# sean-lo/OptimalMatrixCompletion.jl

Measured on AMD Instinct MI355X. Metric: B&B node-relaxations/sec, 100x100 k=1, higher is better.
Workload: dtype f64

## Files before the change

optimalmatrixcompletion.jl_amd/csrc/omc_api.cpp:

```cpp
#include <hip/hip_runtime.h>
#include <stdint.h>
#include <limits.h>
#include <stdio.h>
#include <stdlib.h>
#include <string.h>
#include <math.h>
#include <chrono>
#include <string>
#include <vector>
#include <algorithm>
#include <atomic>
#include <thread>
#include <mutex>

#include "omc.h"
#include "omc_device.h"
#include "omc_altmin.h"
#include "omc_shor.h"
#include "omc_shor_relax.h"
#include <unordered_map>
#include <dlfcn.h>
#include <execinfo.h>
#include <signal.h>
#include <unistd.h>
// ... 35 lines not shown
  p->eps_gap = 1e-6; p->eps_feas = 1e-7; p->max_iters = 3000; p->check_every = 25;
  p->rho_scale = 1.0; p->rho_f_ratio = 0.1; p->relax = 1.6; p->time_limit = 3600.0;
  p->reference_quirk_q1 = 1; p->breakpoints = OMC_SMALLEST_1_EIGVEC; p->stall_checks = 8;
  p->bump_max = 2; p->bump_ratio = 4.0; p->bump_factor = 4.0; p->bump_after = 100; p->bump_window = 4; p->slots = 0;
  p->accel = 0; p->aa_mem = 10; p->aa_every = 10; p->aa_start = 50; p->aa_reg = 1e-10; p->aa_safeguard = 1.0; p->first_wins = 0;
  p->early_stop_after = 400; p->early_stop_factor = 1.5;
}

static int upload(DevBuf& b, const void* src, size_t bytes, hipStream_t s) {
  int rc = b.ensure(bytes ? bytes : 8);
  if (rc) return rc;
  if (bytes) HIPCHK(hipMemcpyAsync(b.p, src, bytes, hipMemcpyHostToDevice, s));
  return 0;
}

static int build_colprox_lists(omc_instance* h, int block_min, bool pair_on) {
  if (h->lists_valid && h->lists_block_min == block_min && h->lists_pair == pair_on) return 0;
  const int m = h->m, lds_c = cp_block_lds_cmax(), max_c = cp_block_cmax();
  std::vector<int> solo, wide, blk, slab;
  std::vector<uint8_t> isb(m, 0);
  h->cpb_cl = h->cpb_cs = h->crest_max = h->nrest = 0;
  for (int j0 = 0; j0 < m; j0 += 2) {
    const int j1 = j0 + 1;
    const int c0 = h->col_ptr[j0 + 1] - h->col_ptr[j0], c1 = (j1 < m) ? h->col_ptr[j1 + 1] - h->col_ptr[j1] : 0;
    const bool paired = j1 < m && c0 <= 32 && c1 <= 32;
    for (int j = j0; j <= j1 && j < m; ++j) {
      const int c = (j == j0) ? c0 : c1;
      if (c == 0) continue;
      if (!(paired && pair_on) && c >= block_min && c <= max_c) {
        isb[j] = 1;
        if (c <= lds_c) { blk.push_back(j); h->cpb_cl = std::max(h->cpb_cl, c); } else { slab.push_back(j); h->cpb_cs = std::max(h->cpb_cs, c); }
        continue;
      }
      ++h->nrest; h->crest_max = std::max(h->crest_max, c);
      if (paired) continue;
      if (c <= 64) wide.push_back(j); else solo.push_back(j);
    }
  }
  h->nsolo = (int)solo.size(); h->nwide = (int)wide.size(); h->nblock = (int)blk.size(); h->nslab = (int)slab.size();
  int rc = 0;
  if (h->nsolo && (rc = upload(h->dsolo, solo.data(), sizeof(int) * solo.size(), h->stream))) return rc;
  if (h->nwide && (rc = upload(h->dwide, wide.data(), sizeof(int) * wide.size(), h->stream))) return rc;
  if (h->nblock && (rc = upload(h->dblock, blk.data(), sizeof(int) * blk.size(), h->stream))) return rc;
  if (h->nslab && (rc = upload(h->dslab, slab.data(), sizeof(int) * slab.size(), h->stream))) return rc;
  if ((rc = upload(h->disblock, isb.data(), (size_t)m, h->stream))) return rc;
  HIPCHK(hipStreamSynchronize(h->stream));
  h->lists_valid = true; h->lists_block_min = block_min; h->lists_pair = pair_on;
  return 0;
}

int omc_instance_create(int n, int m, int k, const double* A, const uint8_t* mask, double gamma, int device,
                        omc_instance** out) {
  if (!out) return fail(OMC_ERR_ARGUMENT, "out is NULL");
  *out = nullptr;
  if (!A || !mask) return fail(OMC_ERR_ARGUMENT, "A / mask is NULL");
  if (n <= 0 || m <= 0) return fail(OMC_ERR_DIMENSION, "Dimension mismatch: A must have size (n, m) (OMC.jl:240-246)");
  if (!(n <= m)) return fail(OMC_ERR_DIMENSION, "Input matrix A must have size (n, m) with n <= m (OMC.jl:249-254)");
  if (k < 1 || k > n) return fail(OMC_ERR_ARGUMENT, "rank k must satisfy 1 <= k <= n");
  if (k > 8) return fail(OMC_ERR_UNSUPPORTED, "k > 8 is not supported by this build");
  if (!(gamma > 0.0)) return fail(OMC_ERR_ARGUMENT, "gamma must be positive");
  int ndev = 0;
  if (hipGetDeviceCount(&ndev) != hipSuccess || ndev <= 0)
// ... 28 lines not shown
  h->row_ptr.assign(n + 1, 0);
  for (int i = 0; i < n; ++i) {
    int c = 0;
    for (int j = 0; j < m; ++j)
      if (h->mask[(size_t)j * n + i]) { h->row_idx.push_back(j); h->row_val.push_back(A[(size_t)j * n + i]); ++c; }
    h->row_ptr[i + 1] = h->row_ptr[i] + c;
  }
  HIPCHK(hipStreamCreate(&h->stream));
  int rc = 0;
  if ((rc = upload(h->drow_ptr, h->row_ptr.data(), sizeof(int) * (n + 1), h->stream))) return rc;
  if ((rc = upload(h->drow_idx, h->row_idx.data(), sizeof(int) * h->nnz_rows(), h->stream))) return rc;
  if ((rc = upload(h->drow_val, h->row_val.data(), sizeof(double) * h->nnz_rows(), h->stream))) return rc;
  if ((rc = upload(h->dA, h->A.data(), sizeof(double) * n * m, h->stream))) return rc;
  if ((rc = upload(h->dmask, h->mask.data(), (size_t)n * m, h->stream))) return rc;
  if ((rc = upload(h->dcol_ptr, h->col_ptr.data(), sizeof(int) * (m + 1), h->stream))) return rc;
  if ((rc = build_colprox_lists(h, h->tun.colprox_block_min, !h->tun.no_colprox_pair))) return rc;
  if ((rc = upload(h->dcol_idx, h->col_idx.data(), sizeof(int) * h->nnz, h->stream))) return rc;
  if ((rc = upload(h->dcol_val, h->col_val.data(), sizeof(double) * h->nnz, h->stream))) return rc;
  if ((rc = upload(h->dNcnt, h->Ncnt.data(), sizeof(double) * n * n, h->stream))) return rc;
  HIPCHK(hipStreamSynchronize(h->stream));
  int lrc = omc_set_max_lds();
  if (lrc) return fail(lrc, "hipFuncSetAttribute(MaxDynamicSharedMemorySize) failed");
  { int arc = omc_altmin_set_lds(); if (arc) return fail(5000 + arc, "hipFuncSetAttribute(MaxDynamicSharedMemorySize) failed for the altmin kernel"); }
  omc_relax_params_default(&h->params);
  *out = h;
  h = nullptr;
  return 0;
}

int omc_instance_create_bits(int n, int m, int k, const double* A, const uint64_t* chunks, double gamma, int device,
                             omc_instance** out) {
// ... 261 lines not shown
    int r0 = h->bgap.ensure(sizeof(double) * 2 * (size_t)S); if (r0) return r0;
    r0 = h->bvotes.ensure(sizeof(int) * (size_t)S); if (r0) return r0;
    r0 = h->bslotlist.ensure(sizeof(int) * (size_t)S); if (r0) return r0;
    w.gap_prev = h->bgap.as<double>(); w.gap_rate = h->bgap.as<double>() + S; w.slow_votes = h->bvotes.as<int>();
    w.slot_list = nullptr;
  }
  std::vector<double> wY((size_t)n * n);
  for (size_t e = 0; e < (size_t)n * n; ++e) wY[e] = shor ? 3.0 : P.rho_f_ratio * h->Ncnt[e] + 2.0;
  int rc_ = 0;
  if ((rc_ = upload(h->dwY, wY.data(), sizeof(double) * n * n, h->stream))) return rc_;
  w.col_ptr = h->dcol_ptr.as<int>(); w.col_idx = h->dcol_idx.as<int>(); w.col_val = h->dcol_val.as<double>();
  const int cp_force = h->cp_force;
  h->cp_force = 0;
  {
    const bool pair_on = !h->tun.no_colprox_pair && cp_force != 2;
    if ((rc_ = build_colprox_lists(h, cp_force == 1 ? INT_MAX : cp_force == 2 ? 1 : h->tun.colprox_block_min, pair_on))) return rc_;
    w.cp_pair = pair_on ? 1 : 0;
  }
  w.cp_nblock = h->nblock; w.cp_block = h->nblock ? h->dblock.as<int>() : nullptr;
  w.cp_nslab = h->nslab; w.cp_slab = h->nslab ? h->dslab.as<int>() : nullptr;
  w.cp_isblock = (h->nblock + h->nslab) ? h->disblock.as<unsigned char>() : nullptr; w.cp_nrest = h->nrest; w.cp_nfact = nullptr;
  w.cone_512 = h->tun.cone_512 ? 1 : 0; w.cp_series = CP_SERIES; w.cp_maxpass = CP_MAXPASS; w.cp_xcd = h->tun.colprox_no_xcd ? 0 : 1;
  w.cp_nsolo = h->nsolo; w.cp_solo = h->nsolo ? h->dsolo.as<int>() : nullptr;
  w.cp_nwide = h->nwide; w.cp_wide = h->nwide ? h->dwide.as<int>() : nullptr;
  w.Ncnt = h->dNcnt.as<double>(); w.wY1 = h->dwY.as<double>();
  w.row_ptr = h->drow_ptr.as<int>(); w.row_idx = h->drow_idx.as<int>();
#define ENS(buf, bytes) do { int r_ = (buf).ensure(bytes); if (r_) return r_; } while (0)
  const size_t sB = (size_t)S;
  const size_t sN = (size_t)B + (size_t)extra_nodes;
  ENS(h->bY, sB * n * n * 8); ENS(h->bYp, sB * n * n * 8); ENS(h->bU, sB * n * k * 8);
  ENS(h->bD1, sB * n * n * 8); ENS(h->bD3, sB * n * n * 8); ENS(h->bW1, sB * n * n * 8); ENS(h->bE3, sB * n * n * 8);
  ENS(h->bdS, sB * rmax * rmax * 8);
// ... 1864 lines not shown
```

optimalmatrixcompletion.jl_amd/csrc/omc_colprox.hip:

```cpp
#include <hip/hip_runtime.h>
#include <type_traits>
#include <stdint.h>
#include "omc_device.h"
#include "omc_wave.h"

template <int Q>
__device__ __forceinline__ double half_bcast(double v) {
  int lo = __double2loint(v), hi = __double2hiint(v);
  lo = __builtin_amdgcn_update_dpp(0, lo, 0x150 + (Q & 15), 0xF, 0xF, false);
  hi = __builtin_amdgcn_update_dpp(0, hi, 0x150 + (Q & 15), 0xF, 0xF, false);
  auto a = __builtin_amdgcn_permlane16_swap(lo, lo, false, false);
  auto c = __builtin_amdgcn_permlane16_swap(hi, hi, false, false);
  return (Q < 16) ? __hiloint2double(c[0], a[0]) : __hiloint2double(c[1], a[1]);
}
__device__ __forceinline__ double half_sum(double v) {
  v = group_sum_dpp<16>(v);
  const int lo = __double2loint(v), hi = __double2hiint(v);
  auto a = __builtin_amdgcn_permlane16_swap(lo, lo, false, false);
  auto c = __builtin_amdgcn_permlane16_swap(hi, hi, false, false);
  return __hiloint2double(c[0], a[0]) + __hiloint2double(c[1], a[1]);
}
#define CPP_LDS_DOUBLES (64 + 64 + 32)

template <int LPC>
__device__ __forceinline__ double lanes_sum(double v) { if constexpr (LPC == 32) return half_sum(v); else return wave_sum(v); }
#define RQ(q) (((q) < 32) ? R0[(q) & 31] : R1[((NC > 32) ? (q) : 0) & 31])
typedef double dbl2_lds __attribute__((ext_vector_type(2), may_alias));
template <int LPC>
__device__ __forceinline__ void colprox_sweep(const OmcWS& w, const int b, const int lane, const int j, const int off, const int c, const int cmax,
                                              double* st, double* vo_s, int* sidx) {
  constexpr int NC = LPC;
  const int h = (LPC == 32) ? (lane >> 5) : 0, l = lane & (LPC - 1), hb = h * LPC;
  const bool act = l < c;
  const int n = w.n;
  const double gm = w.gamma;
  const double* Y = w.Y + (size_t)b * n * n;
  const double* Yp = w.Yp + (size_t)b * n * n;
  const double* Yx = w.Yx ? w.Yx + (size_t)b * n * n : nullptr;
  double* alpha = w.alpha + (size_t)b * w.nnz + off;
  const double a_reg = act ? w.col_val[off + l] : 0.0;
  const int my = act ? w.col_idx[off + l] : 0;
  const double vo_r = act ? alpha[l] : 0.0;
  sidx[lane] = my; vo_s[lane] = vo_r;
  const double rho_f = w.rho_b[b] * w.rho_f_ratio;
  const double coef = gm / (2.0 * rho_f), cp = gm * gm / (2.0 * rho_f);
  double R0[32], R1[(NC > 32) ? 32 : 1], sc;
  const dbl2_lds* st2 = (const dbl2_lds*)st;
  auto gather = [&](double shift) __attribute__((always_inline)) {
#pragma unroll
    for (int qb = 0; qb < NC; qb += 8) {
      if (qb < cmax) {
        double y1[8], y2[8], vq[8];
#pragma unroll
        for (int u = 0; u < 8; ++u) {
          const int iq = sidx[hb + qb + u];
          vq[u] = vo_s[hb + qb + u];
          const size_t a = (l > qb + u) ? (size_t)iq * n + my : (size_t)my * n + iq;
          y1[u] = Yx ? Yx[a] : Y[a]; y2[u] = Yx ? 0.0 : Yp[a];
        }
#pragma unroll
        for (int u = 0; u < 8; ++u) {
          const int q = qb + u;
          const double v = gm * ((Yx ? y1[u] : 2.0 * y1[u] - y2[u]) - coef * vo_r * vq[u]);
          RQ(q) = (l == q) ? (act ? v + 1.0 : 1.0) + shift : ((act && q < c) ? v : 0.0);
        }
      } else {
#pragma unroll
        for (int u = 0; u < 8; ++u) RQ(qb + u) = 0.0;
      }
    }
  };
  auto invert = [&]() __attribute__((always_inline)) -> bool {
    int cm = cmax;
    asm volatile("" : "+s"(cm));
    int lv = l;
    asm volatile("" : "+v"(lv));
    sc = 1.0;
    double isc = 1.0;
    bool good = true;
#pragma unroll
    for (int k = 0; k < NC; ++k) {
      if (k < cm) {
        const double ak = RQ(k) * sc;
        st[lane] = ak;
        const double d = st[hb + k];
        good = good && (d > 1e-290);
        const double pinv = fast_rcp(d);
        const bool piv = (lv == k);
        const double tt = piv ? 0.0 : ak * pinv * isc;
#pragma unroll
        for (int qb = 0; qb < NC; qb += 4) {
          if (qb < cm) {
            if constexpr (LPC == 32) {
              const dbl2_lds s01 = st2[(hb + qb) >> 1], s23 = st2[((hb + qb) >> 1) + 1];
              if (qb != k) RQ(qb) = fma(-tt, s01.x, RQ(qb));
              if (qb + 1 != k) RQ(qb + 1) = fma(-tt, s01.y, RQ(qb + 1));
              if (qb + 2 != k) RQ(qb + 2) = fma(-tt, s23.x, RQ(qb + 2));
              if (qb + 3 != k) RQ(qb + 3) = fma(-tt, s23.y, RQ(qb + 3));
            } else {
#pragma unroll
              for (int u = 0; u < 4; ++u) {
                const int q = qb + u;
                if (q != k) RQ(q) = fma(-tt, st[hb + q], RQ(q));
              }
            }
          }
        }
        RQ(k) = piv ? -1.0 : tt;
        sc = piv ? pinv : sc;
        isc = piv ? d : isc;
      }
    }
    return good;
  };
  auto apply = [&](double v) __attribute__((always_inline)) -> double {
    int cm = cmax;
    asm volatile("" : "+s"(cm));
    st[lane] = v;
    double a0 = 0.0, a1 = 0.0, a2 = 0.0, a3 = 0.0;
#pragma unroll
    for (int qb = 0; qb < NC; qb += 4) {
      if (qb < cm) {
        if constexpr (LPC == 32) {
          const dbl2_lds s01 = st2[(hb + qb) >> 1], s23 = st2[((hb + qb) >> 1) + 1];
          a0 = fma(RQ(qb), s01.x, a0); a1 = fma(RQ(qb + 1), s01.y, a1);
          a2 = fma(RQ(qb + 2), s23.x, a2); a3 = fma(RQ(qb + 3), s23.y, a3);
        } else {
          a0 = fma(RQ(qb), st[hb + qb], a0); a1 = fma(RQ(qb + 1), st[hb + qb + 1], a1);
          a2 = fma(RQ(qb + 2), st[hb + qb + 2], a2); a3 = fma(RQ(qb + 3), st[hb + qb + 3], a3);
        }
      }
    }
    return -sc * ((a0 + a1) + (a2 + a3));
  };
  const double sprev = (j < w.m) ? w.sval[(size_t)b * w.m + j] : 0.0;
  double s = (sprev > 0.0) ? sprev : 0.0;
  double lo = 0.0, hi = -1.0;
  bool lo_valid = false, fin = (c == 0);
  double yout = 0.0;
  const double ser_lim = (w.cp_series >= 6) ? 5e-3 : 1e-5;
  int npass = 0; double dr_first = -1.0; int why = 0;
  for (int it = 0; it <= 60; ++it) {
    if (!__any(!fin)) break;
    const bool last = (it >= w.cp_maxpass);
    gather(cp * s);
    const bool ok_ = invert();
    if (!fin) ++npass;
    double v[6] = {0.0, 0.0, 0.0, 0.0, 0.0, 0.0};
    double rhs = a_reg, yy = 0.0, yz = 0.0, zz = 0.0;
    bool want_ser = false; double dstep = 0.0;
    int K = 2;
    for (int sv = 0; sv < K; ++sv) {
      const double x = apply(rhs);
      rhs = x;
#pragma unroll
      for (int q = 0; q < 6; ++q) v[q] = (sv == q) ? x : v[q];
      if (sv == 0 && last) { if (!fin) { yout = x; fin = true; } break; }
      if (sv == 1) {
        yy = lanes_sum<LPC>(v[0] * v[0]); yz = lanes_sum<LPC>(v[0] * v[1]); zz = lanes_sum<LPC>(v[1] * v[1]);
        bool big = false;
        if (!fin) {
          if (!ok_) {
            lo = s; lo_valid = false;
            s = (hi > 0.0) ? 0.5 * (s + hi) : (2.0 * s + 1.0);
          } else {
            const double ph = yy - s, dph = -2.0 * cp * yz - 1.0, ddph = 6.0 * cp * cp * zz;
            if (ph >= 0.0) { lo = s; lo_valid = true; } else { hi = s; }
            const double den = 2.0 * dph * dph - ph * ddph;
            double sn = s + ((den > dph * dph) ? (-2.0 * ph * dph / den) : (-ph / dph));
            bool guarded = false;
            if (!(sn > lo) && !lo_valid) { sn = 0.5 * (lo + s); guarded = true; }
            if (sn < lo) { sn = lo; guarded = true; }
            if (hi > 0.0 && sn > hi) { sn = 0.5 * (lo + hi); guarded = true; }
            const double d = sn - s;
            const double dr = (yy > 0.0) ? cp * fabs(d) * sqrt(zz / yy) : 1.0;
            if (dr_first < 0.0) { dr_first = dr; why = guarded ? 1 : 0; }
            if (fabs(d) <= 1e-13 * fmax(1.0, fabs(s))) { fin = true; yout = v[0]; }
            else if (!guarded && dr < ser_lim) { want_ser = true; dstep = d; big = dr >= 1e-5; }
            else s = sn;
          }
        }
        if (__any(want_ser)) K = __any(want_ser && big) ? 6 : 3;
      }
    }
    if (K > 2) {
      double mo[13];
      mo[2] = yy; mo[3] = yz; mo[4] = zz;
#pragma unroll
      for (int i = 2; i < 6; ++i) {
        if (i < K) { mo[2 * i + 1] = lanes_sum<LPC>(v[i - 1] * v[i]); mo[2 * i + 2] = lanes_sum<LPC>(v[i] * v[i]); }
        else { mo[2 * i + 1] = 0.0; mo[2 * i + 2] = 0.0; }
      }
      if (want_ser) {
        double cf[11];
#pragma unroll
        for (int p = 2; p <= 12; ++p) {
          const int cnt = (p <= K + 1) ? p - 1 : ((p <= 2 * K) ? 2 * K - p + 1 : 0);
          cf[p - 2] = (double)cnt * mo[p];
        }
        double d = dstep;
        bool conv = false;
        for (int nt = 0; nt < 8; ++nt) {
          const double t = -cp * d;
          double G = 0.0, dG = 0.0;
#pragma unroll
          for (int q = 10; q >= 0; --q) { dG = fma(dG, t, G); G = fma(G, t, cf[q]); }
          const double F = G - s - d, dF = -cp * dG - 1.0;
          const double dn = d - F / dF;
          conv = fabs(dn - d) <= 1e-14 * fmax(fabs(s), fabs(dn));
          d = dn;
          if (conv) break;
        }
        const double t = cp * d;
        const double t2 = t * t;
        const double lastterm = ((K == 6) ? t2 * t2 * fabs(t) : t2) * sqrt(fmax((K == 6) ? mo[12] : mo[6], 0.0));
        const double growth = sqrt(fmax((K == 6) ? mo[12] : mo[6], 0.0) / fmax((K == 6) ? mo[10] : mo[4], 1e-300));
        if (conv && s + d > lo * (lo_valid ? 1.0 : 0.0) && lastterm * fabs(t) * growth <= 2e-15 * sqrt(yy) && fabs(t) * growth < 0.05) {
          double acc = 0.0;
#pragma unroll
          for (int q = 5; q >= 0; --q) acc = (q < K) ? fma(acc, -t, v[q]) : acc;
          yout = acc; s = s + d; fin = true;
        } else {
          s = s + dstep;
        }
      }
    }
  }
  if (w.sub_debug == 4 && l == 0 && c > 0) {
    atomicAdd(&w.stamps[(npass < 7) ? npass : 7], 1.0);
    if (dr_first >= 0.0) { const int bin = (dr_first > 0.0) ? (int)fmin(15.0, fmax(0.0, -log10(dr_first))) : 15; atomicAdd(&w.stamps[8 + bin], 1.0); if (why) atomicAdd(&w.stamps[24], 1.0); }
    else atomicAdd(&w.stamps[25], 1.0);
  }
  if (act) {
    alpha[l] = yout;
    w.lamD[((size_t)b * w.m + j) * n + my] = yout;
    if (l == 0) w.sval[(size_t)b * w.m + j] = s;
  }
}


#undef RQ
__global__ void __launch_bounds__(256) __attribute__((amdgpu_waves_per_eu(3))) k_colprox_pair(OmcWS w) {
  extern __shared__ double smem[];
  const int wave_in_blk = __builtin_amdgcn_readfirstlane(threadIdx.x >> 6), lane = threadIdx.x & 63, wpb = blockDim.x >> 6;
  const int gw = xcd_block(w.cp_xcd) * wpb + wave_in_blk;
  const int mp = (w.m + 1) >> 1;
  const int bl = gw / mp, pr = gw - bl * mp;
  if (bl >= w.nB) return;
  const int b = slot_of(w, bl);
  if (w.done[b]) return;
  const int j0 = 2 * pr, j1 = j0 + 1;
  const int off0 = w.col_ptr[j0], c0 = w.col_ptr[j0 + 1] - off0;
  const int off1 = (j1 < w.m) ? w.col_ptr[j1] : 0, c1 = (j1 < w.m) ? w.col_ptr[j1 + 1] - off1 : 0;
  if (c0 > 32 || c1 > 32 || j1 >= w.m) return;
  const int cmax = __builtin_amdgcn_readfirstlane((c0 > c1) ? c0 : c1);
  if (cmax == 0) return;
  double* st = smem + (size_t)wave_in_blk * CPP_LDS_DOUBLES;
  double* vo_s = st + 64;
  int* sidx = (int*)(vo_s + 64);
  const int h = lane >> 5;
  colprox_sweep<32>(w, b, lane, j0 + h, h ? off1 : off0, h ? c1 : c0, cmax, st, vo_s, sidx);
}

__global__ void __launch_bounds__(256) __attribute__((amdgpu_waves_per_eu(2))) k_colprox_wide(OmcWS w) {
  extern __shared__ double smem[];
  const int wave_in_blk = __builtin_amdgcn_readfirstlane(threadIdx.x >> 6), lane = threadIdx.x & 63, wpb = blockDim.x >> 6;
  const int gw = xcd_block(w.cp_xcd) * wpb + wave_in_blk;
  const int bl = gw / w.cp_nwide, jj = gw - bl * w.cp_nwide;
  if (bl >= w.nB) return;
  const int b = slot_of(w, bl);
  if (w.done[b]) return;
  const int j = w.cp_wide[jj];
  const int off = w.col_ptr[j], c = w.col_ptr[j + 1] - off;
  const int cmax = __builtin_amdgcn_readfirstlane(c);
  if (cmax == 0 || cmax > 64) return;
  double* st = smem + (size_t)wave_in_blk * CPP_LDS_DOUBLES;
  double* vo_s = st + 64;
  int* sidx = (int*)(vo_s + 64);
  colprox_sweep<64>(w, b, lane, j, off, c, cmax, st, vo_s, sidx);
}


extern "C" void omc_launch_colprox_sweep(const OmcWS* w, hipStream_t s) {
  const int wpb = 4;
  const int wp = w->nB * ((w->m + 1) / 2);
  hipLaunchKernelGGL(k_colprox_pair, dim3((wp + wpb - 1) / wpb), dim3(wpb * 64), (size_t)wpb * CPP_LDS_DOUBLES * sizeof(double), s, *w);
  if (w->cp_nwide > 0) {
    const int ww = w->nB * w->cp_nwide;
    hipLaunchKernelGGL(k_colprox_wide, dim3((ww + wpb - 1) / wpb), dim3(wpb * 64), (size_t)wpb * CPP_LDS_DOUBLES * sizeof(double), s, *w);
  }
}

extern "C" void omc_colprox_sweep_residency(int* pair, int* wide) {
  const int wpb = 4;
  const size_t lds = (size_t)wpb * CPP_LDS_DOUBLES * sizeof(double);
  if (hipOccupancyMaxActiveBlocksPerMultiprocessor(pair, (const void*)k_colprox_pair, wpb * 64, lds) != hipSuccess) *pair = -1;
  if (hipOccupancyMaxActiveBlocksPerMultiprocessor(wide, (const void*)k_colprox_wide, wpb * 64, lds) != hipSuccess) *wide = -1;
}
```

optimalmatrixcompletion.jl_amd/csrc/omc_device.h:

```cpp
#ifndef OMC_DEVICE_H
#define OMC_DEVICE_H
#include <hip/hip_runtime.h>
#include <stdint.h>

#define ROW_TRACE 0
#define ROW_BOX 1
#define ROW_BOUND 2
#define ROW_CUT 3

#define CONE_CLIP01 0
#define CONE_EVALS 2
#define CONE_SEP 3
#define CONE_TOPK 4
#define CONE_BIG 5
#define SMALL_PROJ 0
#define SMALL_RECOVER 1

#define OMC_ST_OPTIMAL 0
#define OMC_ST_SLOW 1
#define OMC_ST_TIME 2
#define OMC_ST_INFEASIBLE 3

#include "omc_layout.h"

// ... 66 lines not shown
  int *rkind, *rcut, *rbi, *rbj;
  double* rcoef;
  double* rrhs;
  double* cutx;
  double* G;
  int setup_gram_inline;
  double* lam;
  double *obj, *objout, *objprev, *lbprev, *lb, *c0, *evsum, *cpen, *cst, *rp, *rd, *lmin;
  double* bx;
  int *done, *status, *iters, *sweeps, *stall;
  int* rowov;
  OmcGeom geo;
  double* cp_scratch;
  int cp_pair; int cp_nsolo; const int* cp_solo;
  int cp_nwide; const int* cp_wide;
  int cp_nrest;
  int cp_nblock, cp_nslab; const int *cp_block, *cp_slab; const unsigned char* cp_isblock; double* cp_bslab; int* cp_nfact;
  double* Yx;
  int cone_512;
  int cp_series;
  int cp_maxpass;
  int cp_xcd;
  double *cone_scratch, *glob_scratch, *small_scratch;
  double* chk_scratch;
  double* stamps;
  int accel, aa_mem, aa_every, aa_start, aa_dim;
  double aa_reg, aa_safeguard;
  double *aa_F, *aa_G, *aa_zin;
  double* aa_fn;
  int *aa_hist, *aa_head, *aa_pending, *aa_valid, *aa_nacc, *aa_nrej;
// ... 40 lines not shown
```

optimalmatrixcompletion.jl_amd/csrc/omc_host.h:

```cpp
#pragma once
#include <hip/hip_runtime.h>
#include <stdint.h>
#include <atomic>
#include <mutex>
#include <string>
#include <thread>
#include <unordered_map>
#include <vector>

#include "omc.h"
#include "omc_device.h"
#include "omc_shor_relax.h"

extern thread_local std::string g_err;
static inline int fail(int code, const std::string& msg) { g_err = msg; return code; }
#define HIPCHK(x)                                                                                         \
  do {                                                                                                    \
    hipError_t e_ = (x);                                                                                  \
    if (e_ != hipSuccess) {                                                                               \
      g_err = std::string(#x) + ": " + hipGetErrorString(e_);                                             \
      return (int)e_ > 0 ? (int)e_ : 999;                                                                 \
    }                                                                                                     \
  } while (0)

// ... 40 lines not shown
  bool colprox_no_xcd = false;
  bool cone_512 = false;
  bool dense_proj = false;
  bool host_phases = false;
  bool global_nolds = false;
  bool no_colprox_pair = false;
  bool no_graph = false;
  bool no_subspace = false;
  bool no_ws_split = false;
  bool segv_trace = false;
  bool setup_gram_inline = false;
  bool shor_explicit = false;
  bool shor_no_subspace = false;
  int check_xs = 16;
  int colprox_block_min = 65;
  int cone_multi_min = 1025;
  int graph_max = 16;
  int harvest_async = 1;
  int harvest_async_min_live = 256;
  int shor_select_kb = 1048576;
  int streams = 4;
  int sub_debug = 0;
  int sub_qmax = 24;
  int timing_stride = 1;
  int ws_quiet = 1;
};
struct Knob { const char* name; bool Tuning::*flag; int Tuning::*num; };
inline const Knob OMC_KNOBS[] = {
  {"OMC_ALTMIN_NOLDS", &Tuning::altmin_nolds, nullptr},      {"OMC_COLPROX_NO_XCD", &Tuning::colprox_no_xcd, nullptr},
  {"OMC_CONE_512", &Tuning::cone_512, nullptr},              {"OMC_DENSE_PROJ", &Tuning::dense_proj, nullptr},
  {"OMC_GLOBAL_NOLDS", &Tuning::global_nolds, nullptr},      {"OMC_HOST_PHASES", &Tuning::host_phases, nullptr},
  {"OMC_NO_COLPROX_PAIR", &Tuning::no_colprox_pair, nullptr},
  {"OMC_NO_GRAPH", &Tuning::no_graph, nullptr},              {"OMC_NO_SUBSPACE", &Tuning::no_subspace, nullptr},
  {"OMC_NO_WS_SPLIT", &Tuning::no_ws_split, nullptr},        {"OMC_SEGV_TRACE", &Tuning::segv_trace, nullptr},
  {"OMC_SETUP_GRAM_INLINE", &Tuning::setup_gram_inline, nullptr},
  {"OMC_SHOR_EXPLICIT", &Tuning::shor_explicit, nullptr},    {"OMC_SHOR_NO_SUBSPACE", &Tuning::shor_no_subspace, nullptr},
  {"OMC_COLPROX_BLOCK_MIN", nullptr, &Tuning::colprox_block_min},
  {"OMC_CHECK_XS", nullptr, &Tuning::check_xs},              {"OMC_CONE_MULTI_MIN", nullptr, &Tuning::cone_multi_min},
  {"OMC_GRAPH_MAX", nullptr, &Tuning::graph_max},            {"OMC_SHOR_SELECT_KB", nullptr, &Tuning::shor_select_kb},
  {"OMC_HARVEST_ASYNC", nullptr, &Tuning::harvest_async},    {"OMC_HARVEST_ASYNC_MIN_LIVE", nullptr, &Tuning::harvest_async_min_live},
  {"OMC_WS_QUIET", nullptr, &Tuning::ws_quiet},
  {"OMC_STREAMS", nullptr, &Tuning::streams},
  {"OMC_SUB_DEBUG", nullptr, &Tuning::sub_debug},            {"OMC_SUB_QMAX", nullptr, &Tuning::sub_qmax},
  {"OMC_TIMING_STRIDE", nullptr, &Tuning::timing_stride},
};

struct omc_instance {
  int n = 0, m = 0, k = 0, device = 0, nnz = 0, cmax = 0;
  double gamma = 0, sumA2 = 0;
  std::vector<int> col_ptr, col_idx; std::vector<double> col_val;
  std::vector<double> A; std::vector<uint8_t> mask;
  std::vector<double> Ncnt;
  std::vector<int> row_ptr, row_idx; std::vector<double> row_val;
  DevBuf drow_ptr, drow_idx, drow_val, aR, arkind, arcut, arbi, arbj, arcoef, arrhs, acutx, aU0, aU, aV, aobj, aint, aG, aG2;
  hipStream_t stream = nullptr;
  Tuning tun;
  hipStream_t gs[3] = {};
  hipEvent_t gev[5] = {};
  hipEvent_t gevc[5] = {};
  hipEvent_t ev_main = nullptr;
  PinBuf pin_flags[2], pin_list[2], pin_done, pin_jobs; DevBuf bgramjobs;
  hipEvent_t ev_up[4] = {}; bool ev_up_rec[4] = {}; hipEvent_t ev_gram = nullptr; bool ev_gram_rec = false;
  double host_ms[OMC_HOST_NPHASE] = {0}; int64_t host_cnt[OMC_HOST_NPHASE] = {0};
  DevBuf dA, dmask, dcol_ptr, dcol_idx, dcol_val, dNcnt, dwY, dsolo, dwide;
  int nwide = 0;
  int nsolo = 0;
  DevBuf dblock, dslab, disblock, bcpb, bnfact;
  int nblock = 0, nslab = 0, nrest = 0, cpb_cl = 0, cpb_cs = 0, crest_max = 0;
  bool lists_valid = false; int lists_block_min = 0; bool lists_pair = true;
  int cp_force = 0;
  DevBuf bYx, bY, bYp, bU, bD1, bD3, bW1, bE3, bQb, brr, bsm, bdS, balpha, balphaX, bsval, bMchk, bsmall, bchk;
  DevBuf bR, brkind, brcut, brbi, brbj, brcoef, brrhs, bcutx, bG, blam;
  DevBuf bobjcol, baaF, baaG, baaZ, baaS, baaI, bMbufC, bVrowC, bchkS, bchkI;
  DevBuf bslotlist, bgap, bvotes, blamDX, bXsC, bsubSC, bsubIC;
  DevBuf bsubz, bscal, bbx, bint, bcp, bcone, bglob, bXout, bThout, bXin, bMbuf, bVrow, bXs, bsubS, bsubI;
  long long sub_tot[8] = {0};
  DevBuf bmwstat, sbigmw, pjM, pjV, pjW, pjS, pjD, pjI;
  long long mw_tot[5] = {0};
  OmcWS ws{};
  omc_relax_params params{};
  bool staged = false;
  double last_solve_seconds = 0; long long total_sweeps = 0; int last_iters_total = 0;
  std::thread worker; std::atomic<int> worker_running{0}, nodes_done{0}; int worker_rc = 0; std::string worker_err;
  int reserve_nodes = 0, reserve_cuts = 0, node_cap = 0, staged_cut_type = 0; std::atomic<int> Btot_live{0}; bool append_closed = true; std::mutex append_mu; hipStream_t append_stream = nullptr;
// ... 48 lines not shown
```

Baseline: 2287.

## Pack four small columns per wave with two rows per lane in colprox

Adds a quad colprox kernel that processes four paired columns (each ≤32 entries) per 64-lane wave, with 16 lanes per column and two rows per lane. Column pairs are sorted by size so columns of similar length share a wave, and any leftover pair goes to the existing pair kernel. The aim is to halve the number of waves for small columns and cut wasted lanes, at the cost of more registers per lane. The gather arithmetic is also rewritten with explicit non-contracted multiplies and adds so results match the rounding of the original code. The path is on by default through OMC_COLPROX_QUAD.

```diff
diff --git a/optimalmatrixcompletion.jl_amd/csrc/omc_api.cpp b/optimalmatrixcompletion.jl_amd/csrc/omc_api.cpp
--- a/optimalmatrixcompletion.jl_amd/csrc/omc_api.cpp
+++ b/optimalmatrixcompletion.jl_amd/csrc/omc_api.cpp
@@ -73,16 +73,19 @@
   return 0;
 }
 
-static int build_colprox_lists(omc_instance* h, int block_min, bool pair_on) {
-  if (h->lists_valid && h->lists_block_min == block_min && h->lists_pair == pair_on) return 0;
+static int build_colprox_lists(omc_instance* h, int block_min, bool pair_on, bool quad_on) {
+  quad_on = quad_on && pair_on;
+  if (h->lists_valid && h->lists_block_min == block_min && h->lists_pair == pair_on && h->lists_quad == quad_on) return 0;
   const int m = h->m, lds_c = cp_block_lds_cmax(), max_c = cp_block_cmax();
-  std::vector<int> solo, wide, blk, slab;
+  std::vector<int> solo, wide, blk, slab, quad, pairl;
+  std::vector<std::pair<int, int>> pairs;
   std::vector<uint8_t> isb(m, 0);
   h->cpb_cl = h->cpb_cs = h->crest_max = h->nrest = 0;
   for (int j0 = 0; j0 < m; j0 += 2) {
     const int j1 = j0 + 1;
     const int c0 = h->col_ptr[j0 + 1] - h->col_ptr[j0], c1 = (j1 < m) ? h->col_ptr[j1 + 1] - h->col_ptr[j1] : 0;
     const bool paired = j1 < m && c0 <= 32 && c1 <= 32;
+    if (paired && quad_on && std::max(c0, c1) > 0) pairs.push_back({std::max(c0, c1), j0 / 2});
     for (int j = j0; j <= j1 && j < m; ++j) {
       const int c = (j == j0) ? c0 : c1;
       if (c == 0) continue;
@@ -96,15 +99,22 @@
       if (c <= 64) wide.push_back(j); else solo.push_back(j);
     }
   }
+  std::stable_sort(pairs.begin(), pairs.end(), [](const std::pair<int, int>& a, const std::pair<int, int>& b) { return a.first > b.first; });
+  for (size_t i = 0; i + 1 < pairs.size(); i += 2)
+    for (int u = 0; u < 2; ++u) { quad.push_back(2 * pairs[i + u].second); quad.push_back(2 * pairs[i + u].second + 1); }
+  if (pairs.size() & 1) pairl.push_back(pairs.back().second);
+  h->nquad = (int)quad.size() / 4; h->npairl = (int)pairl.size();
   h->nsolo = (int)solo.size(); h->nwide = (int)wide.size(); h->nblock = (int)blk.size(); h->nslab = (int)slab.size();
   int rc = 0;
+  if (h->nquad && (rc = upload(h->dquad, quad.data(), sizeof(int) * quad.size(), h->stream))) return rc;
+  if (h->npairl && (rc = upload(h->dpairl, pairl.data(), sizeof(int) * pairl.size(), h->stream))) return rc;
   if (h->nsolo && (rc = upload(h->dsolo, solo.data(), sizeof(int) * solo.size(), h->stream))) return rc;
   if (h->nwide && (rc = upload(h->dwide, wide.data(), sizeof(int) * wide.size(), h->stream))) return rc;
   if (h->nblock && (rc = upload(h->dblock, blk.data(), sizeof(int) * blk.size(), h->stream))) return rc;
   if (h->nslab && (rc = upload(h->dslab, slab.data(), sizeof(int) * slab.size(), h->stream))) return rc;
   if ((rc = upload(h->disblock, isb.data(), (size_t)m, h->stream))) return rc;
   HIPCHK(hipStreamSynchronize(h->stream));
-  h->lists_valid = true; h->lists_block_min = block_min; h->lists_pair = pair_on;
+  h->lists_valid = true; h->lists_block_min = block_min; h->lists_pair = pair_on; h->lists_quad = quad_on;
   return 0;
 }
 
@@ -163,7 +173,7 @@
   if ((rc = upload(h->dA, h->A.data(), sizeof(double) * n * m, h->stream))) return rc;
   if ((rc = upload(h->dmask, h->mask.data(), (size_t)n * m, h->stream))) return rc;
   if ((rc = upload(h->dcol_ptr, h->col_ptr.data(), sizeof(int) * (m + 1), h->stream))) return rc;
-  if ((rc = build_colprox_lists(h, h->tun.colprox_block_min, !h->tun.no_colprox_pair))) return rc;
+  if ((rc = build_colprox_lists(h, h->tun.colprox_block_min, !h->tun.no_colprox_pair, h->tun.colprox_quad != 0))) return rc;
   if ((rc = upload(h->dcol_idx, h->col_idx.data(), sizeof(int) * h->nnz, h->stream))) return rc;
   if ((rc = upload(h->dcol_val, h->col_val.data(), sizeof(double) * h->nnz, h->stream))) return rc;
   if ((rc = upload(h->dNcnt, h->Ncnt.data(), sizeof(double) * n * n, h->stream))) return rc;
@@ -455,8 +465,11 @@
   h->cp_force = 0;
   {
     const bool pair_on = !h->tun.no_colprox_pair && cp_force != 2;
-    if ((rc_ = build_colprox_lists(h, cp_force == 1 ? INT_MAX : cp_force == 2 ? 1 : h->tun.colprox_block_min, pair_on))) return rc_;
+    if ((rc_ = build_colprox_lists(h, cp_force == 1 ? INT_MAX : cp_force == 2 ? 1 : h->tun.colprox_block_min, pair_on, h->tun.colprox_quad != 0))) return rc_;
     w.cp_pair = pair_on ? 1 : 0;
+    w.cp_quad = (pair_on && h->tun.colprox_quad != 0) ? 1 : 0;
+    w.cp_nquad = h->nquad; w.cp_quadl = h->nquad ? h->dquad.as<int>() : nullptr;
+    w.cp_npairl = h->npairl; w.cp_pairl = h->npairl ? h->dpairl.as<int>() : nullptr;
   }
   w.cp_nblock = h->nblock; w.cp_block = h->nblock ? h->dblock.as<int>() : nullptr;
   w.cp_nslab = h->nslab; w.cp_slab = h->nslab ? h->dslab.as<int>() : nullptr;
diff --git a/optimalmatrixcompletion.jl_amd/csrc/omc_colprox.hip b/optimalmatrixcompletion.jl_amd/csrc/omc_colprox.hip
--- a/optimalmatrixcompletion.jl_amd/csrc/omc_colprox.hip
+++ b/optimalmatrixcompletion.jl_amd/csrc/omc_colprox.hip
@@ -21,52 +21,86 @@
   return __hiloint2double(c[0], a[0]) + __hiloint2double(c[1], a[1]);
 }
 #define CPP_LDS_DOUBLES (64 + 64 + 32)
+#define CPQ_COL_STRIDE 34
+#define CPQ_LDS_DOUBLES (4 * CPQ_COL_STRIDE + 128 + 64)
 
 template <int LPC>
 __device__ __forceinline__ double lanes_sum(double v) { if constexpr (LPC == 32) return half_sum(v); else return wave_sum(v); }
-#define RQ(q) (((q) < 32) ? R0[(q) & 31] : R1[((NC > 32) ? (q) : 0) & 31])
+template <int LPC, int RPL>
+__device__ __forceinline__ double col_sum(const double (&p)[RPL]) {
+  if constexpr (RPL == 2) return group_sum_dpp<16>(p[0]) + group_sum_dpp<16>(p[1]); else return lanes_sum<LPC>(p[0]);
+}
+__device__ __forceinline__ double mul_rn(double a, double b) {
+#pragma clang fp contract(off)
+  return a * b;
+}
+__device__ __forceinline__ double add_rn(double a, double b) {
+#pragma clang fp contract(off)
+  return a + b;
+}
+#define RQ(r, q) ((RPL == 2) ? (((r) == 0) ? R0[(q) & 31] : R1[(q) & 31]) : (((q) < 32) ? R0[(q) & 31] : R1[((NC > 32) ? (q) : 0) & 31]))
 typedef double dbl2_lds __attribute__((ext_vector_type(2), may_alias));
-template <int LPC>
+template <int LPC, int RPL = 1>
 __device__ __forceinline__ void colprox_sweep(const OmcWS& w, const int b, const int lane, const int j, const int off, const int c, const int cmax,
                                               double* st, double* vo_s, int* sidx) {
-  constexpr int NC = LPC;
-  const int h = (LPC == 32) ? (lane >> 5) : 0, l = lane & (LPC - 1), hb = h * LPC;
-  const bool act = l < c;
+  constexpr int NC = LPC * RPL;
+  constexpr int CST = (RPL == 2) ? CPQ_COL_STRIDE : LPC;
+  static_assert(RPL == 1 || (RPL == 2 && LPC == 16), "two rows per lane: 16 lanes per column");
+  const int h = (LPC == 64) ? 0 : (lane / LPC), l = lane & (LPC - 1), hb = h * CST, vb = h * NC;
+  bool act[RPL];
+#pragma unroll
+  for (int r = 0; r < RPL; ++r) act[r] = l + r * LPC < c;
   const int n = w.n;
   const double gm = w.gamma;
   const double* Y = w.Y + (size_t)b * n * n;
   const double* Yp = w.Yp + (size_t)b * n * n;
   const double* Yx = w.Yx ? w.Yx + (size_t)b * n * n : nullptr;
   double* alpha = w.alpha + (size_t)b * w.nnz + off;
-  const double a_reg = act ? w.col_val[off + l] : 0.0;
-  const int my = act ? w.col_idx[off + l] : 0;
-  const double vo_r = act ? alpha[l] : 0.0;
-  sidx[lane] = my; vo_s[lane] = vo_r;
+  double a_reg[RPL], vo_r[RPL]; int my[RPL];
+#pragma unroll
+  for (int r = 0; r < RPL; ++r) {
+    const int row = l + r * LPC;
+    a_reg[r] = act[r] ? w.col_val[off + row] : 0.0;
+    my[r] = act[r] ? w.col_idx[off + row] : 0;
+    vo_r[r] = act[r] ? alpha[row] : 0.0;
+    sidx[vb + row] = my[r]; vo_s[vb + row] = vo_r[r];
+  }
   const double rho_f = w.rho_b[b] * w.rho_f_ratio;
   const double coef = gm / (2.0 * rho_f), cp = gm * gm / (2.0 * rho_f);
-  double R0[32], R1[(NC > 32) ? 32 : 1], sc;
+  double R0[32], R1[(NC > 32 || RPL == 2) ? 32 : 1], sc[RPL];
   const dbl2_lds* st2 = (const dbl2_lds*)st;
   auto gather = [&](double shift) __attribute__((always_inline)) {
 #pragma unroll
     for (int qb = 0; qb < NC; qb += 8) {
       if (qb < cmax) {
-        double y1[8], y2[8], vq[8];
+        double y1[RPL][8], y2[RPL][8], vq[8];
 #pragma unroll
         for (int u = 0; u < 8; ++u) {
-          const int iq = sidx[hb + qb + u];
-          vq[u] = vo_s[hb + qb + u];
-          const size_t a = (l > qb + u) ? (size_t)iq * n + my : (size_t)my * n + iq;
-          y1[u] = Yx ? Yx[a] : Y[a]; y2[u] = Yx ? 0.0 : Yp[a];
-        }
-#pragma unroll
-        for (int u = 0; u < 8; ++u) {
-          const int q = qb + u;
-          const double v = gm * ((Yx ? y1[u] : 2.0 * y1[u] - y2[u]) - coef * vo_r * vq[u]);
-          RQ(q) = (l == q) ? (act ? v + 1.0 : 1.0) + shift : ((act && q < c) ? v : 0.0);
+          const int iq = sidx[vb + qb + u];
+          vq[u] = vo_s[vb + qb + u];
+#pragma unroll
+          for (int r = 0; r < RPL; ++r) {
+            const size_t a = (l + r * LPC > qb + u) ? (size_t)iq * n + my[r] : (size_t)my[r] * n + iq;
+            y1[r][u] = Yx ? Yx[a] : Y[a]; y2[r][u] = Yx ? 0.0 : Yp[a];
+          }
+        }
+#pragma unroll
+        for (int r = 0; r < RPL; ++r) {
+#pragma unroll
+          for (int u = 0; u < 8; ++u) {
+            const int q = qb + u;
+            const double x = fma(-mul_rn(coef, vo_r[r]), vq[u], Yx ? y1[r][u] : fma(y1[r][u], 2.0, -y2[r][u]));
+            const double v = mul_rn(gm, x);
+            const double dg = (u == 7) ? add_rn(v, 1.0) : fma(gm, x, 1.0);
+            RQ(r, q) = (l + r * LPC == q) ? add_rn(act[r] ? dg : 1.0, shift) : ((act[r] && q < c) ? v : 0.0);
+          }
         }
       } else {
 #pragma unroll
-        for (int u = 0; u < 8; ++u) RQ(qb + u) = 0.0;
+        for (int r = 0; r < RPL; ++r) {
+#pragma unroll
+          for (int u = 0; u < 8; ++u) RQ(r, qb + u) = 0.0;
+        }
       }
     }
   };
@@ -75,69 +109,98 @@
     asm volatile("" : "+s"(cm));
     int lv = l;
     asm volatile("" : "+v"(lv));
-    sc = 1.0;
-    double isc = 1.0;
+    double isc[RPL];
+#pragma unroll
+    for (int r = 0; r < RPL; ++r) { sc[r] = 1.0; isc[r] = 1.0; }
     bool good = true;
 #pragma unroll
     for (int k = 0; k < NC; ++k) {
       if (k < cm) {
-        const double ak = RQ(k) * sc;
-        st[lane] = ak;
+        double ak[RPL];
+#pragma unroll
+        for (int r = 0; r < RPL; ++r) ak[r] = RQ(r, k) * sc[r];
+        if constexpr (RPL == 1) st[lane] = ak[0];
+        else {
+#pragma unroll
+          for (int r = 0; r < RPL; ++r) st[hb + l + r * LPC] = ak[r];
+        }
         const double d = st[hb + k];
         good = good && (d > 1e-290);
         const double pinv = fast_rcp(d);
-        const bool piv = (lv == k);
-        const double tt = piv ? 0.0 : ak * pinv * isc;
+        bool piv[RPL]; double tt[RPL];
+#pragma unroll
+        for (int r = 0; r < RPL; ++r) {
+          piv[r] = (r == k / LPC) && (lv == (k & (LPC - 1)));
+          tt[r] = piv[r] ? 0.0 : ak[r] * pinv * isc[r];
+        }
 #pragma unroll
         for (int qb = 0; qb < NC; qb += 4) {
           if (qb < cm) {
-            if constexpr (LPC == 32) {
+            if constexpr (LPC != 64) {
               const dbl2_lds s01 = st2[(hb + qb) >> 1], s23 = st2[((hb + qb) >> 1) + 1];
-              if (qb != k) RQ(qb) = fma(-tt, s01.x, RQ(qb));
-              if (qb + 1 != k) RQ(qb + 1) = fma(-tt, s01.y, RQ(qb + 1));
-              if (qb + 2 != k) RQ(qb + 2) = fma(-tt, s23.x, RQ(qb + 2));
-              if (qb + 3 != k) RQ(qb + 3) = fma(-tt, s23.y, RQ(qb + 3));
+#pragma unroll
+              for (int r = 0; r < RPL; ++r) {
+                if (qb != k) RQ(r, qb) = fma(-tt[r], s01.x, RQ(r, qb));
+                if (qb + 1 != k) RQ(r, qb + 1) = fma(-tt[r], s01.y, RQ(r, qb + 1));
+                if (qb + 2 != k) RQ(r, qb + 2) = fma(-tt[r], s23.x, RQ(r, qb + 2));
+                if (qb + 3 != k) RQ(r, qb + 3) = fma(-tt[r], s23.y, RQ(r, qb + 3));
+              }
             } else {
 #pragma unroll
               for (int u = 0; u < 4; ++u) {
                 const int q = qb + u;
-                if (q != k) RQ(q) = fma(-tt, st[hb + q], RQ(q));
+                if (q != k) RQ(0, q) = fma(-tt[0], st[hb + q], RQ(0, q));
               }
             }
           }
         }
-        RQ(k) = piv ? -1.0 : tt;
-        sc = piv ? pinv : sc;
-        isc = piv ? d : isc;
+#pragma unroll
+        for (int r = 0; r < RPL; ++r) {
+          RQ(r, k) = piv[r] ? -1.0 : tt[r];
+          sc[r] = piv[r] ? pinv : sc[r];
+          isc[r] = piv[r] ? d : isc[r];
+        }
       }
     }
     return good;
   };
-  auto apply = [&](double v) __attribute__((always_inline)) -> double {
+  auto apply = [&](const double (&v)[RPL], double (&x)[RPL]) __attribute__((always_inline)) {
     int cm = cmax;
     asm volatile("" : "+s"(cm));
-    st[lane] = v;
-    double a0 = 0.0, a1 = 0.0, a2 = 0.0, a3 = 0.0;
+    if constexpr (RPL == 1) st[lane] = v[0];
+    else {
+#pragma unroll
+      for (int r = 0; r < RPL; ++r) st[hb + l + r * LPC] = v[r];
+    }
+    double a0[RPL], a1[RPL], a2[RPL], a3[RPL];
+#pragma unroll
+    for (int r = 0; r < RPL; ++r) { a0[r] = 0.0; a1[r] = 0.0; a2[r] = 0.0; a3[r] = 0.0; }
 #pragma unroll
     for (int qb = 0; qb < NC; qb += 4) {
       if (qb < cm) {
-        if constexpr (LPC == 32) {
+        if constexpr (LPC != 64) {
           const dbl2_lds s01 = st2[(hb + qb) >> 1], s23 = st2[((hb + qb) >> 1) + 1];
-          a0 = fma(RQ(qb), s01.x, a0); a1 = fma(RQ(qb + 1), s01.y, a1);
-          a2 = fma(RQ(qb + 2), s23.x, a2); a3 = fma(RQ(qb + 3), s23.y, a3);
+#pragma unroll
+          for (int r = 0; r < RPL; ++r) {
+            a0[r] = fma(RQ(r, qb), s01.x, a0[r]); a1[r] = fma(RQ(r, qb + 1), s01.y, a1[r]);
+            a2[r] = fma(RQ(r, qb + 2), s23.x, a2[r]); a3[r] = fma(RQ(r, qb + 3), s23.y, a3[r]);
+          }
         } else {
-          a0 = fma(RQ(qb), st[hb + qb], a0); a1 = fma(RQ(qb + 1), st[hb + qb + 1], a1);
-          a2 = fma(RQ(qb + 2), st[hb + qb + 2], a2); a3 = fma(RQ(qb + 3), st[hb + qb + 3], a3);
-        }
-      }
-    }
-    return -sc * ((a0 + a1) + (a2 + a3));
+          a0[0] = fma(RQ(0, qb), st[hb + qb], a0[0]); a1[0] = fma(RQ(0, qb + 1), st[hb + qb + 1], a1[0]);
+          a2[0] = fma(RQ(0, qb + 2), st[hb + qb + 2], a2[0]); a3[0] = fma(RQ(0, qb + 3), st[hb + qb + 3], a3[0]);
+        }
+      }
+    }
+#pragma unroll
+    for (int r = 0; r < RPL; ++r) x[r] = -sc[r] * ((a0[r] + a1[r]) + (a2[r] + a3[r]));
   };
   const double sprev = (j < w.m) ? w.sval[(size_t)b * w.m + j] : 0.0;
   double s = (sprev > 0.0) ? sprev : 0.0;
   double lo = 0.0, hi = -1.0;
   bool lo_valid = false, fin = (c == 0);
-  double yout = 0.0;
+  double yout[RPL];
+#pragma unroll
+  for (int r = 0; r < RPL; ++r) yout[r] = 0.0;
   const double ser_lim = (w.cp_series >= 6) ? 5e-3 : 1e-5;
   int npass = 0; double dr_first = -1.0; int why = 0;
   for (int it = 0; it <= 60; ++it) {
@@ -146,18 +209,39 @@
     gather(cp * s);
     const bool ok_ = invert();
     if (!fin) ++npass;
-    double v[6] = {0.0, 0.0, 0.0, 0.0, 0.0, 0.0};
-    double rhs = a_reg, yy = 0.0, yz = 0.0, zz = 0.0;
+    double v[6][RPL];
+#pragma unroll
+    for (int q = 0; q < 6; ++q) {
+#pragma unroll
+      for (int r = 0; r < RPL; ++r) v[q][r] = 0.0;
+    }
+    double rhs[RPL], yy = 0.0, yz = 0.0, zz = 0.0;
+#pragma unroll
+    for (int r = 0; r < RPL; ++r) rhs[r] = a_reg[r];
     bool want_ser = false; double dstep = 0.0;
-    int K = 2;
+    int K = 2, Kq = 2;
     for (int sv = 0; sv < K; ++sv) {
-      const double x = apply(rhs);
-      rhs = x;
-#pragma unroll
-      for (int q = 0; q < 6; ++q) v[q] = (sv == q) ? x : v[q];
-      if (sv == 0 && last) { if (!fin) { yout = x; fin = true; } break; }
+      double x[RPL];
+      apply(rhs, x);
+#pragma unroll
+      for (int r = 0; r < RPL; ++r) {
+        rhs[r] = x[r];
+#pragma unroll
+        for (int q = 0; q < 6; ++q) v[q][r] = (sv == q) ? x[r] : v[q][r];
+      }
+      if (sv == 0 && last) {
+        if (!fin) {
+#pragma unroll
+          for (int r = 0; r < RPL; ++r) yout[r] = x[r];
+          fin = true;
+        }
+        break;
+      }
       if (sv == 1) {
-        yy = lanes_sum<LPC>(v[0] * v[0]); yz = lanes_sum<LPC>(v[0] * v[1]); zz = lanes_sum<LPC>(v[1] * v[1]);
+        double p00[RPL], p01[RPL], p11[RPL];
+#pragma unroll
+        for (int r = 0; r < RPL; ++r) { p00[r] = v[0][r] * v[0][r]; p01[r] = v[0][r] * v[1][r]; p11[r] = v[1][r] * v[1][r]; }
+        yy = col_sum<LPC, RPL>(p00); yz = col_sum<LPC, RPL>(p01); zz = col_sum<LPC, RPL>(p11);
         bool big = false;
         if (!fin) {
           if (!ok_) {
@@ -175,27 +259,45 @@
             const double d = sn - s;
             const double dr = (yy > 0.0) ? cp * fabs(d) * sqrt(zz / yy) : 1.0;
             if (dr_first < 0.0) { dr_first = dr; why = guarded ? 1 : 0; }
-            if (fabs(d) <= 1e-13 * fmax(1.0, fabs(s))) { fin = true; yout = v[0]; }
+            if (fabs(d) <= 1e-13 * fmax(1.0, fabs(s))) {
+              fin = true;
+#pragma unroll
+              for (int r = 0; r < RPL; ++r) yout[r] = v[0][r];
+            }
             else if (!guarded && dr < ser_lim) { want_ser = true; dstep = d; big = dr >= 1e-5; }
             else s = sn;
           }
         }
-        if (__any(want_ser)) K = __any(want_ser && big) ? 6 : 3;
-      }
-    }
+        if constexpr (RPL == 2) {
+          const unsigned long long ws = __ballot(want_ser), wb = __ballot(want_ser && big);
+          const unsigned hs = (unsigned)(lane < 32 ? ws : ws >> 32), hg = (unsigned)(lane < 32 ? wb : wb >> 32);
+          if (hs) Kq = hg ? 6 : 3;
+          if (ws) K = wb ? 6 : 3;
+        } else {
+          if (__any(want_ser)) K = __any(want_ser && big) ? 6 : 3;
+        }
+      }
+    }
+    const int Kh = (RPL == 2) ? Kq : K;
     if (K > 2) {
       double mo[13];
       mo[2] = yy; mo[3] = yz; mo[4] = zz;
 #pragma unroll
       for (int i = 2; i < 6; ++i) {
-        if (i < K) { mo[2 * i + 1] = lanes_sum<LPC>(v[i - 1] * v[i]); mo[2 * i + 2] = lanes_sum<LPC>(v[i] * v[i]); }
+        if (i < K) {
+          double pa[RPL], pb[RPL];
+#pragma unroll
+          for (int r = 0; r < RPL; ++r) { pa[r] = v[i - 1][r] * v[i][r]; pb[r] = v[i][r] * v[i][r]; }
+          const double sa = col_sum<LPC, RPL>(pa), sb = col_sum<LPC, RPL>(pb);
+          mo[2 * i + 1] = (i < Kh) ? sa : 0.0; mo[2 * i + 2] = (i < Kh) ? sb : 0.0;
+        }
         else { mo[2 * i + 1] = 0.0; mo[2 * i + 2] = 0.0; }
       }
       if (want_ser) {
         double cf[11];
 #pragma unroll
         for (int p = 2; p <= 12; ++p) {
-          const int cnt = (p <= K + 1) ? p - 1 : ((p <= 2 * K) ? 2 * K - p + 1 : 0);
+          const int cnt = (p <= Kh + 1) ? p - 1 : ((p <= 2 * Kh) ? 2 * Kh - p + 1 : 0);
           cf[p - 2] = (double)cnt * mo[p];
         }
         double d = dstep;
@@ -213,13 +315,17 @@
         }
         const double t = cp * d;
         const double t2 = t * t;
-        const double lastterm = ((K == 6) ? t2 * t2 * fabs(t) : t2) * sqrt(fmax((K == 6) ? mo[12] : mo[6], 0.0));
-        const double growth = sqrt(fmax((K == 6) ? mo[12] : mo[6], 0.0) / fmax((K == 6) ? mo[10] : mo[4], 1e-300));
+        const double lastterm = ((Kh == 6) ? t2 * t2 * fabs(t) : t2) * sqrt(fmax((Kh == 6) ? mo[12] : mo[6], 0.0));
+        const double growth = sqrt(fmax((Kh == 6) ? mo[12] : mo[6], 0.0) / fmax((Kh == 6) ? mo[10] : mo[4], 1e-300));
         if (conv && s + d > lo * (lo_valid ? 1.0 : 0.0) && lastterm * fabs(t) * growth <= 2e-15 * sqrt(yy) && fabs(t) * growth < 0.05) {
-          double acc = 0.0;
-#pragma unroll
-          for (int q = 5; q >= 0; --q) acc = (q < K) ? fma(acc, -t, v[q]) : acc;
-          yout = acc; s = s + d; fin = true;
+#pragma unroll
+          for (int r = 0; r < RPL; ++r) {
+            double acc = 0.0;
+#pragma unroll
+            for (int q = 5; q >= 0; --q) acc = (q < Kh) ? fma(acc, -t, v[q][r]) : acc;
+            yout[r] = acc;
+          }
+          s = s + d; fin = true;
         } else {
           s = s + dstep;
         }
@@ -231,10 +337,13 @@
     if (dr_first >= 0.0) { const int bin = (dr_first > 0.0) ? (int)fmin(15.0, fmax(0.0, -log10(dr_first))) : 15; atomicAdd(&w.stamps[8 + bin], 1.0); if (why) atomicAdd(&w.stamps[24], 1.0); }
     else atomicAdd(&w.stamps[25], 1.0);
   }
-  if (act) {
-    alpha[l] = yout;
-    w.lamD[((size_t)b * w.m + j) * n + my] = yout;
-    if (l == 0) w.sval[(size_t)b * w.m + j] = s;
+#pragma unroll
+  for (int r = 0; r < RPL; ++r) {
+    if (act[r]) {
+      alpha[l + r * LPC] = yout[r];
+      w.lamD[((size_t)b * w.m + j) * n + my[r]] = yout[r];
+      if (l + r * LPC == 0) w.sval[(size_t)b * w.m + j] = s;
+    }
   }
 }
 
@@ -244,11 +353,12 @@
   extern __shared__ double smem[];
   const int wave_in_blk = __builtin_amdgcn_readfirstlane(threadIdx.x >> 6), lane = threadIdx.x & 63, wpb = blockDim.x >> 6;
   const int gw = xcd_block(w.cp_xcd) * wpb + wave_in_blk;
-  const int mp = (w.m + 1) >> 1;
-  const int bl = gw / mp, pr = gw - bl * mp;
+  const int mp = w.cp_quad ? w.cp_npairl : (w.m + 1) >> 1;
+  const int bl = gw / mp, pi = gw - bl * mp;
   if (bl >= w.nB) return;
   const int b = slot_of(w, bl);
   if (w.done[b]) return;
+  const int pr = w.cp_quad ? w.cp_pairl[pi] : pi;
   const int j0 = 2 * pr, j1 = j0 + 1;
   const int off0 = w.col_ptr[j0], c0 = w.col_ptr[j0 + 1] - off0;
   const int off1 = (j1 < w.m) ? w.col_ptr[j1] : 0, c1 = (j1 < w.m) ? w.col_ptr[j1 + 1] - off1 : 0;
@@ -260,6 +370,28 @@
   int* sidx = (int*)(vo_s + 64);
   const int h = lane >> 5;
   colprox_sweep<32>(w, b, lane, j0 + h, h ? off1 : off0, h ? c1 : c0, cmax, st, vo_s, sidx);
+}
+
+__global__ void __launch_bounds__(256) __attribute__((amdgpu_waves_per_eu(2))) k_colprox_quad(OmcWS w) {
+  extern __shared__ double smem[];
+  const int wave_in_blk = __builtin_amdgcn_readfirstlane(threadIdx.x >> 6), lane = threadIdx.x & 63, wpb = blockDim.x >> 6;
+  const int gw = xcd_block(w.cp_xcd) * wpb + wave_in_blk;
+  const int bl = gw / w.cp_nquad, g = gw - bl * w.cp_nquad;
+  if (bl >= w.nB) return;
+  const int b = slot_of(w, bl);
+  if (w.done[b]) return;
+  const int* jq = w.cp_quadl + 4 * g;
+  int cm = 0;
+#pragma unroll
+  for (int u = 0; u < 4; ++u) { const int ju = jq[u], cu = w.col_ptr[ju + 1] - w.col_ptr[ju]; cm = (cu > cm) ? cu : cm; }
+  const int cmax = __builtin_amdgcn_readfirstlane(cm);
+  if (cmax == 0 || cmax > 32) return;
+  double* st = smem + (size_t)wave_in_blk * CPQ_LDS_DOUBLES;
+  double* vo_s = st + 4 * CPQ_COL_STRIDE;
+  int* sidx = (int*)(vo_s + 128);
+  const int j = jq[lane >> 4];
+  const int off = w.col_ptr[j], c = w.col_ptr[j + 1] - off;
+  colprox_sweep<16, 2>(w, b, lane, j, off, c, cmax, st, vo_s, sidx);
 }
 
 __global__ void __launch_bounds__(256) __attribute__((amdgpu_waves_per_eu(2))) k_colprox_wide(OmcWS w) {
@@ -283,8 +415,12 @@
 
 extern "C" void omc_launch_colprox_sweep(const OmcWS* w, hipStream_t s) {
   const int wpb = 4;
-  const int wp = w->nB * ((w->m + 1) / 2);
-  hipLaunchKernelGGL(k_colprox_pair, dim3((wp + wpb - 1) / wpb), dim3(wpb * 64), (size_t)wpb * CPP_LDS_DOUBLES * sizeof(double), s, *w);
+  if (w->cp_quad && w->cp_nquad > 0) {
+    const int wq = w->nB * w->cp_nquad;
+    hipLaunchKernelGGL(k_colprox_quad, dim3((wq + wpb - 1) / wpb), dim3(wpb * 64), (size_t)wpb * CPQ_LDS_DOUBLES * sizeof(double), s, *w);
+  }
+  const int wp = w->nB * (w->cp_quad ? w->cp_npairl : (w->m + 1) / 2);
+  if (wp > 0) hipLaunchKernelGGL(k_colprox_pair, dim3((wp + wpb - 1) / wpb), dim3(wpb * 64), (size_t)wpb * CPP_LDS_DOUBLES * sizeof(double), s, *w);
   if (w->cp_nwide > 0) {
     const int ww = w->nB * w->cp_nwide;
     hipLaunchKernelGGL(k_colprox_wide, dim3((ww + wpb - 1) / wpb), dim3(wpb * 64), (size_t)wpb * CPP_LDS_DOUBLES * sizeof(double), s, *w);
diff --git a/optimalmatrixcompletion.jl_amd/csrc/omc_device.h b/optimalmatrixcompletion.jl_amd/csrc/omc_device.h
--- a/optimalmatrixcompletion.jl_amd/csrc/omc_device.h
+++ b/optimalmatrixcompletion.jl_amd/csrc/omc_device.h
@@ -104,6 +104,7 @@
   double* cp_scratch;
   int cp_pair; int cp_nsolo; const int* cp_solo;
   int cp_nwide; const int* cp_wide;
+  int cp_quad; int cp_nquad; const int* cp_quadl; int cp_npairl; const int* cp_pairl;
   int cp_nrest;
   int cp_nblock, cp_nslab; const int *cp_block, *cp_slab; const unsigned char* cp_isblock; double* cp_bslab; int* cp_nfact;
   double* Yx;
diff --git a/optimalmatrixcompletion.jl_amd/csrc/omc_host.h b/optimalmatrixcompletion.jl_amd/csrc/omc_host.h
--- a/optimalmatrixcompletion.jl_amd/csrc/omc_host.h
+++ b/optimalmatrixcompletion.jl_amd/csrc/omc_host.h
@@ -78,6 +78,7 @@
   bool shor_no_subspace = false;
   int check_xs = 16;
   int colprox_block_min = 65;
+  int colprox_quad = 1;
   int cone_multi_min = 1025;
   int graph_max = 16;
   int harvest_async = 1;
@@ -99,7 +100,7 @@
   {"OMC_NO_WS_SPLIT", &Tuning::no_ws_split, nullptr},        {"OMC_SEGV_TRACE", &Tuning::segv_trace, nullptr},
   {"OMC_SETUP_GRAM_INLINE", &Tuning::setup_gram_inline, nullptr},
   {"OMC_SHOR_EXPLICIT", &Tuning::shor_explicit, nullptr},    {"OMC_SHOR_NO_SUBSPACE", &Tuning::shor_no_subspace, nullptr},
-  {"OMC_COLPROX_BLOCK_MIN", nullptr, &Tuning::colprox_block_min},
+  {"OMC_COLPROX_BLOCK_MIN", nullptr, &Tuning::colprox_block_min}, {"OMC_COLPROX_QUAD", nullptr, &Tuning::colprox_quad},
   {"OMC_CHECK_XS", nullptr, &Tuning::check_xs},              {"OMC_CONE_MULTI_MIN", nullptr, &Tuning::cone_multi_min},
   {"OMC_GRAPH_MAX", nullptr, &Tuning::graph_max},            {"OMC_SHOR_SELECT_KB", nullptr, &Tuning::shor_select_kb},
   {"OMC_HARVEST_ASYNC", nullptr, &Tuning::harvest_async},    {"OMC_HARVEST_ASYNC_MIN_LIVE", nullptr, &Tuning::harvest_async_min_live},
@@ -126,12 +127,13 @@
   PinBuf pin_flags[2], pin_list[2], pin_done, pin_jobs; DevBuf bgramjobs;
   hipEvent_t ev_up[4] = {}; bool ev_up_rec[4] = {}; hipEvent_t ev_gram = nullptr; bool ev_gram_rec = false;
   double host_ms[OMC_HOST_NPHASE] = {0}; int64_t host_cnt[OMC_HOST_NPHASE] = {0};
-  DevBuf dA, dmask, dcol_ptr, dcol_idx, dcol_val, dNcnt, dwY, dsolo, dwide;
+  DevBuf dA, dmask, dcol_ptr, dcol_idx, dcol_val, dNcnt, dwY, dsolo, dwide, dquad, dpairl;
+  int nquad = 0, npairl = 0;
   int nwide = 0;
   int nsolo = 0;
   DevBuf dblock, dslab, disblock, bcpb, bnfact;
   int nblock = 0, nslab = 0, nrest = 0, cpb_cl = 0, cpb_cs = 0, crest_max = 0;
-  bool lists_valid = false; int lists_block_min = 0; bool lists_pair = true;
+  bool lists_valid = false; int lists_block_min = 0; bool lists_pair = true, lists_quad = true;
   int cp_force = 0;
   DevBuf bYx, bY, bYp, bU, bD1, bD3, bW1, bE3, bQb, brr, bsm, bdS, balpha, balphaX, bsval, bMchk, bsmall, bchk;
   DevBuf bR, brkind, brcut, brbi, brbj, brcoef, brrhs, bcutx, bG, blam;
```

Measured after the change: 2349, median of 4. 1.03x the previous value.
